# PX4/disparity_to_point_cloud

Measured on NVIDIA B200. Metric: Mpixels/s disparity->PointCloud2, higher is better.
Workload: dtype f64

## Files before the change

### disparity_to_point_cloud_b200/csrc/capi.cu

```cuda
#include "../../include/d2pc_b200.h"

#include <algorithm>
#include <atomic>
#include <cmath>
#include <cstdio>
#include <cstdlib>
#include <cstring>
#include <mutex>
#include <new>
#include <string>
#include <utility>
#include <vector>

#include <nvtx3/nvToolsExt.h>
#include <sys/mman.h>

#include "cloud_transform.h"
#include "crop_box.h"
#include "fusion.h"
#include "median.h"
#include "radius_outlier.h"
#include "reproject.h"
#include "score.h"
#include "voxel.h"
// ... 54 lines not shown
};

}

struct d2pc_ctx {
  d2pc_config cfg;
  int device = 0;
  int sm_count = 148;
  cudaStream_t s_h2d = nullptr, s_compute = nullptr, s_d2h = nullptr;
  double q[16];
  QParams Q;
  std::vector<Slot> slots;
  uint32_t epoch = 0;
  uint64_t launches = 0;
  std::string last_cuda_error;
  StageBufs batch;
  uint32_t *d_ticket = nullptr;
  d2pc_voxel_grid voxel;
  bool voxel_set = false;
  d2pc_radius_outlier ror;
  d2pc_crop_box box;
  d2pc_cloud_transform xform;
  DevBuf d_fuse_in[4], d_container, d_combined, d_fused;
  PinBuf h_fused, h_combined;
  DevBuf d_score_in, d_score_out[2];
  PinBuf h_score[2];
  DevBuf d_color_in, d_color_out, d_color_lut;
  PinBuf h_color;
  PinBuf h_stage;
  bool color_lut_ready = false;
  cudaEvent_t ev_fuse = nullptr;
  int rows_per_unit = 0, ctas_per_sm = 0, median_strip = 0, median_variant = 0;
  bool force_scalar = false, force_generic = false;
  int compact_variant = 0, exact_variant = 0, prefetch_dist = 0, zero_numer = 0;
  int fuse_median = 0;
  int direct_out = 0;
  bool timing = false;
  std::vector<std::pair<uintptr_t, bool>> pin_cache;
  uint64_t pin_cache_gen = 0;
};

namespace {

struct NvtxRange {
  explicit NvtxRange(const char *name) { nvtxRangePushA(name); }
  ~NvtxRange() { nvtxRangePop(); }
};

std::atomic<uint64_t> g_host_gen{1};

int cuda_fail(d2pc_ctx *ctx, cudaError_t e, const char *what) {
  if (ctx) {
    ctx->last_cuda_error = std::string(what) + ": " + cudaGetErrorString(e);
  }
  if (e == cudaErrorMemoryAllocation) return D2PC_ERR_NOMEM;
  if (e == cudaErrorNoDevice || e == cudaErrorInsufficientDriver || e == cudaErrorInvalidDevice)
    return D2PC_ERR_NO_DEVICE;
  return D2PC_ERR_CUDA;
}

#define CU(ctx, call)                                      \
  do {                                                     \
    cudaError_t e__ = (call);                              \
    if (e__ != cudaSuccess) return cuda_fail(ctx, e__, #call); \
  } while (0)

int grow_dev(d2pc_ctx *ctx, DevBuf &b, size_t bytes, cudaStream_t clear_on = nullptr) {
// ... 266 lines not shown

int enqueue_reproject(d2pc_ctx *ctx, const CloudPlan &p, const FrameBatch &in, StageBufs &b, const CloudDst &dst,
                      uint32_t *ticket, cudaStream_t stream) {
  const d2pc_config &c = ctx->cfg;
  int nl = 0;
  ReprojectLaunch L;
  L.in = in.data;
  L.in_is_f32 = in.is_f32;
  L.step = in.step;
  L.frame_stride = in.frame_stride;
  L.n_frames = in.n_frames;
  L.width = in.w;
  L.height = in.h;
  L.border = c.border;
  L.scale = c.disparity_scale;
  L.out = dst.points;
  L.out_stride_bytes = dst.stride;
  L.counts = dst.counts;
  L.Q = &ctx->Q;
  L.arith_fast = c.arith_mode == D2PC_ARITH_FAST;
  L.compact = p.compact;
  L.scratch = b.scratch.p;
  L.tables = b.tables.p;
  L.ticket = ticket;
  L.sm_count = ctx->sm_count;
  L.rows_per_unit = ctx->rows_per_unit;
  L.ctas_per_sm = ctx->ctas_per_sm;
  L.force_scalar = ctx->force_scalar;
  L.force_generic = ctx->force_generic;
  L.compact_variant = ctx->compact_variant;
  L.exact_variant = ctx->exact_variant;
  L.zero_numer = ctx->zero_numer;
  L.prefetch_dist = ctx->prefetch_dist;
  if (!in.is_f32 && c.median_ksize > 1) {
    MedianLaunch M;
    M.src = in.data;
    M.dst = b.med.p;
    M.src_step = M.dst_step = in.step;
    M.src_frame_stride = M.dst_frame_stride = in.frame_stride;
    M.n_frames = in.n_frames;
    M.width = (int)in.w;
    M.height = (int)in.h;
    M.ox0 = c.border;
    M.oy0 = c.border;
    M.ow = (int)in.w - 2 * c.border;
    M.oh = (int)in.h - 2 * c.border;
    M.ksize = c.median_ksize;
    M.sm_count = ctx->sm_count;
    M.strip_rows = ctx->median_strip;
    M.variant = ctx->median_variant;
    bool zero_numer = false;
    const bool fuse = ctx->fuse_median >= 0 && M.ow > 0 && M.oh > 0 && (c.median_ksize > 3 || M.variant != 0) &&
                      reproject_fuses_with_median(L, &zero_numer);
    if (fuse) {
      M.zero_numer = zero_numer;
      M.points = dst.points;
      M.points_stride_bytes = dst.stride;
      M.Q = &ctx->Q;
      M.scale = c.disparity_scale;
    }
    CU(ctx, launch_median_u8(M, stream, &nl));
    ctx->launches += nl;
    if (fuse) return D2PC_OK;
    L.in = b.med.p;
  }
  L.epoch = L.compact ? next_epoch(ctx) : 0;
// ... 232 lines not shown
  auto fail = [&](int code) {
    d2pc_destroy(ctx);
    return code;
  };
  if (cudaSetDevice(device) != cudaSuccess) return fail(D2PC_ERR_NO_DEVICE);
  cudaDeviceGetAttribute(&ctx->sm_count, cudaDevAttrMultiProcessorCount, device);
  if (cudaStreamCreateWithFlags(&ctx->s_h2d, cudaStreamNonBlocking) != cudaSuccess ||
      cudaStreamCreateWithFlags(&ctx->s_compute, cudaStreamNonBlocking) != cudaSuccess ||
      cudaStreamCreateWithFlags(&ctx->s_d2h, cudaStreamNonBlocking) != cudaSuccess ||
      cudaEventCreateWithFlags(&ctx->ev_fuse, cudaEventDisableTiming) != cudaSuccess)
    return fail(D2PC_ERR_CUDA);
  if (cudaMalloc(&ctx->d_ticket, 64) != cudaSuccess) return fail(D2PC_ERR_NOMEM);
  ctx->slots.resize(c.n_slots);
  for (auto &s : ctx->slots) {
    if (cudaEventCreateWithFlags(&s.ev_h2d, cudaEventDisableTiming) != cudaSuccess ||
        cudaEventCreateWithFlags(&s.ev_kernel, cudaEventDisableTiming) != cudaSuccess ||
        cudaEventCreateWithFlags(&s.ev_d2h, cudaEventDisableTiming) != cudaSuccess ||
        cudaStreamCreateWithFlags(&s.s_kern, cudaStreamNonBlocking) != cudaSuccess)
      return fail(D2PC_ERR_CUDA);
    if (cudaMalloc(&s.d_count, 64) != cudaSuccess) return fail(D2PC_ERR_NOMEM);
    if (cudaHostAlloc(&s.h_count, 64, cudaHostAllocDefault) != cudaSuccess) return fail(D2PC_ERR_NOMEM);
    cudaMemsetAsync(s.d_count, 0, 64, ctx->s_compute);
  }
  rc = d2pc_q_from_intrinsics(c.fx, c.fy, c.cx, c.cy, c.baseline, c.rect_width, c.rect_height, ctx->q);
  if (rc) return fail(rc);
  make_qparams(ctx->q, &ctx->Q);
  d2pc_voxel_grid_default(&ctx->voxel);
  d2pc_radius_outlier_default(&ctx->ror);
  d2pc_crop_box_default(&ctx->box);
  d2pc_cloud_transform_default(&ctx->xform);

  if (const char *v = getenv("D2PC_ROWS_PER_UNIT")) ctx->rows_per_unit = atoi(v);
  if (const char *v = getenv("D2PC_CTAS_PER_SM")) ctx->ctas_per_sm = atoi(v);
  if (const char *v = getenv("D2PC_MEDIAN_STRIP")) ctx->median_strip = atoi(v);
  if (const char *v = getenv("D2PC_EXACT_VARIANT")) ctx->exact_variant = atoi(v);

  if (c.max_width > 0 && c.max_height > 0) {
    for (auto &s : ctx->slots) {
      const size_t pitch = round_up((size_t)c.max_width * 4, kAlign);
      const uint64_t np = crop_points(c.max_width, c.max_height, c.border);
      if ((rc = grow_dev(ctx, s.d_in, pitch * c.max_height)) ||
          (rc = grow_dev(ctx, s.stages.med, pitch * c.max_height)) ||
          (rc = grow_dev(ctx, s.d_out, np * 16 + 16)) || (rc = grow_pin(ctx, s.h_out, np * 16 + 16)) ||
          (rc = grow_pin(ctx, s.h_in, (size_t)c.max_width * 4 * c.max_height)))
        return fail(rc);
    }
  }
  *out = ctx;
  return D2PC_OK;
}

void d2pc_destroy(d2pc_ctx *ctx) {
  if (!ctx) return;
  cudaSetDevice(ctx->device);
  cudaDeviceSynchronize();
  for (auto &s : ctx->slots) {
    free_pin(s.h_in), free_pin(s.h_out);
    free_dev(s.d_in), free_dev(s.d_out), free_stages(s.stages);
    for (auto &b : s.d_fuse_in) free_dev(b);
    free_dev(s.d_pre[0]), free_dev(s.d_pre[1]), free_dev(s.d_container), free_dev(s.d_combined), free_dev(s.d_fused);
    if (s.d_count) cudaFree(s.d_count);
    if (s.h_count) cudaFreeHost(s.h_count);
    if (s.ev_h2d) cudaEventDestroy(s.ev_h2d);
    if (s.ev_kernel) cudaEventDestroy(s.ev_kernel);
    if (s.ev_d2h) cudaEventDestroy(s.ev_d2h);
    if (s.ev_start) cudaEventDestroy(s.ev_start);
// ... 99 lines not shown
}
int d2pc_set_cloud_transform(d2pc_ctx *ctx, const d2pc_cloud_transform *t) {
  if (!ctx || !t || t->struct_size != sizeof(*t)) return D2PC_ERR_INVALID_ARG;
  for (float m : t->matrix)
    if (!std::isfinite(m)) return D2PC_ERR_INVALID_ARG;
  ctx->xform = *t;
  return D2PC_OK;
}
int d2pc_get_cloud_transform(const d2pc_ctx *ctx, d2pc_cloud_transform *t) {
  if (!ctx || !t) return D2PC_ERR_INVALID_ARG;
  *t = ctx->xform;
  return D2PC_OK;
}
int d2pc_set_arith_mode(d2pc_ctx *ctx, int m) {
  if (!ctx || m < 0 || m > 1) return D2PC_ERR_INVALID_ARG;
  ctx->cfg.arith_mode = m;
  return D2PC_OK;
}
int d2pc_set_tuning(d2pc_ctx *ctx, const char *key, int value) {
  if (!ctx || !key) return D2PC_ERR_INVALID_ARG;
  const std::string k(key);
  if (k == "rows_per_unit") ctx->rows_per_unit = value;
  else if (k == "ctas_per_sm") ctx->ctas_per_sm = value;
  else if (k == "median_strip") ctx->median_strip = value;
  else if (k == "median_variant") ctx->median_variant = value;
  else if (k == "force_scalar") ctx->force_scalar = value != 0;
  else if (k == "force_generic") ctx->force_generic = value != 0;
  else if (k == "force_park" || k == "compact_variant") ctx->compact_variant = value;
  else if (k == "exact_variant") ctx->exact_variant = value;
  else if (k == "zero_numer") ctx->zero_numer = value;
  else if (k == "fuse_median") ctx->fuse_median = value;
  else if (k == "direct_out") ctx->direct_out = value;
  else if (k == "prefetch_dist") ctx->prefetch_dist = value;
  else if (k == "median_ksize") {
    if (value < 1 || value > 15 || !(value & 1)) return D2PC_ERR_INVALID_ARG;
    ctx->cfg.median_ksize = value;
  } else if (k == "border") {
    if (value < 0) return D2PC_ERR_INVALID_ARG;
    ctx->cfg.border = value;
  } else if (k == "offset_x") ctx->cfg.offset_x = value;
  else if (k == "offset_y") ctx->cfg.offset_y = value;
  else if (k == "fuse_rule") {
    if (value < 0 || value > 7) return D2PC_ERR_INVALID_ARG;
    ctx->cfg.fuse_rule = value;
  } else if (k == "fuse_median_ksize") {
    if (value < 1 || value > 15 || !(value & 1)) return D2PC_ERR_INVALID_ARG;
    ctx->cfg.fuse_median_ksize = value;
  } else if (k == "fuse_crop_left") ctx->cfg.fuse_crop_left = value;
  else if (k == "fuse_crop_right") ctx->cfg.fuse_crop_right = value;
  else if (k == "fuse_crop_top") ctx->cfg.fuse_crop_top = value;
  else if (k == "fuse_crop_bottom") ctx->cfg.fuse_crop_bottom = value;
  else return D2PC_ERR_INVALID_ARG;
  return D2PC_OK;
}

int d2pc_submit_mono8(d2pc_ctx *ctx, int slot, const uint8_t *data, uint32_t w, uint32_t h, uint32_t step) {
  return submit_common(ctx, slot, data, w, h, step, false);
}
int d2pc_submit_f32(d2pc_ctx *ctx, int slot, const float *disp, uint32_t w, uint32_t h, uint32_t step) {
  return submit_common(ctx, slot, disp, w, h, step, true);
}

int d2pc_wait(d2pc_ctx *ctx, int slot, d2pc_cloud *out) {
  if (!ctx || slot < 0 || slot >= (int)ctx->slots.size()) return D2PC_ERR_INVALID_ARG;
  Slot &s = ctx->slots[slot];
  if (!s.pending) return D2PC_ERR_NOT_READY;
// ... 740 lines not shown
```

### disparity_to_point_cloud_b200/csrc/reproject.cu

```cuda
#include "reproject.h"

#include <algorithm>
#include <cmath>

#include "reproject_math.cuh"

namespace d2pc {

namespace {

constexpr int kWarpsPerCta = 4;
constexpr int kThreads = kWarpsPerCta * 32;
constexpr int kSegCols = 128;

struct FastDiv {
  uint32_t magic, shift;
};
static FastDiv make_fastdiv(uint32_t d) {
  FastDiv f{0u, 0u};
  if (d <= 1) return f;
  uint32_t s = 0;
  while ((1ull << (s + 1)) < d) ++s;
  f.shift = 32 + s;
  f.magic = (uint32_t)(((1ull << f.shift) + d - 1) / d);
  return f;
}
__device__ __forceinline__ uint32_t fastdiv(uint32_t n, FastDiv f) {
  return f.shift == 0u ? n : (uint32_t)(((unsigned long long)n * f.magic) >> f.shift);
}

struct ReprojArgs {
  const uint8_t *in;
  size_t step, frame_stride;
  float4 *out;
  size_t out_frame_stride;
  uint32_t *counts;
  int n_frames, width, height, border, cw, ch;
  int rows_per_unit, n_seg, n_rb;
  uint32_t units_per_frame, total_units;
  FastDiv div_upf, div_nseg;
  float scale;
  unsigned long long *tile_desc;
  uint32_t *ticket;
  uint32_t epoch, tiles_per_frame;
  const double *xtab, *ytab;
  uint32_t d_sure_bits;
  int band_rows, cw_pad, band_groups, group_rows;
  int prefetch_dist;
  QParams Q;
};

enum { kMathRect0 = 0, kMathRectW = 1, kMathGeneric = 2, kMathFast = 3, kMathRect0M = 4, kMathRect0Z = 5 };
#define D2PC_IS_RECT(m) ((m) == kMathRect0 || (m) == kMathRectW || (m) == kMathRect0M || (m) == kMathRect0Z)
#define D2PC_IS_GUARD(m) ((m) == kMathRect0 || (m) == kMathRect0Z)

__device__ __forceinline__ float4 ld_stream_f4(const float4 *p) {
  float4 v;
  asm volatile("ld.global.cs.v4.f32 {%0,%1,%2,%3}, [%4];" : "=f"(v.x), "=f"(v.y), "=f"(v.z), "=f"(v.w) : "l"(p));
  return v;
}
__device__ __forceinline__ void st_stream_f4(float4 *p, const float4 &v) {
  asm volatile("st.global.cs.v4.f32 [%0], {%1,%2,%3,%4};" ::"l"(p), "f"(v.x), "f"(v.y), "f"(v.z), "f"(v.w) : "memory");
}

__device__ __forceinline__ void st_stream_f4_if(float4 *p, const float4 &v, bool pred) {
  asm volatile(
      "{\n\t.reg .pred q;\n\tsetp.ne.b32 q, %5, 0;\n\t@q st.global.cs.v4.f32 [%0], {%1,%2,%3,%4};\n\t}" ::"l"(p),
      "f"(v.x), "f"(v.y), "f"(v.z), "f"(v.w), "r"((int)pred)
      : "memory");
}

__device__ __forceinline__ uint32_t store_ranked(float4 *out, uint32_t pos, const float4 &p, bool keep, int lane,
                                                 uint32_t lt_mask) {
  const uint32_t bal = __ballot_sync(0xffffffffu, keep);
  if (bal == 0xffffffffu) {
    __stcs(out + (pos + (uint32_t)lane), p);
    return pos + 32u;
  }
  if (bal == 0u) return pos;
  if (keep) __stcs(out + (pos + (uint32_t)__popc(bal & lt_mask)), p);
  return pos + (uint32_t)__popc(bal);
}

__device__ __forceinline__ uint32_t store_ranked_tight(float4 *out, uint32_t pos, const float4 &p, bool keep) {
  uint32_t lt;
// ... 37 lines not shown
}

template <int kMath>
__device__ __forceinline__ void points_of4(const QParams &Q, const double (&xd)[4], double yd, uint32_t xslow,
                                           uint32_t yslow, int u0, int v, const float (&d)[4], float4 (&p)[4]) {
  if constexpr (D2PC_IS_RECT(kMath)) {
    bool slow[4];
    const bool ys = (yslow & 1u) != 0u, yz = (yslow & 2u) != 0u;
#pragma unroll
    for (int k = 0; k < 4; ++k) {
      if constexpr (kMath == kMathRect0Z)
        p[k] = reproject_exact_rectified<true, true, true>(Q, xd[k], yd, ys || ((xslow >> k) & 1u),
                                                           yz || ((xslow >> (4 + k)) & 1u), d[k], slow[k]);
      else
        p[k] = reproject_exact_rectified<kMath != kMathRectW, kMath == kMathRect0>(Q, xd[k], yd,
                                                                                   ys || ((xslow >> k) & 1u), false,
                                                                                   d[k], slow[k]);
    }
    if (__builtin_expect(slow[0] || slow[1] || slow[2] || slow[3], 0)) {
#pragma unroll
      for (int k = 0; k < 4; ++k)
        if (slow[k]) p[k] = reproject_exact_slow(Q.q, u0 + 32 * k, v, d[k]);
    }
  } else if constexpr (kMath == kMathGeneric) {
    bool slow[4];
    const double dv = (double)v;
#pragma unroll
    for (int k = 0; k < 4; ++k) p[k] = reproject_exact_generic_guarded(Q.q, (double)(u0 + 32 * k), dv, d[k], slow[k]);
    if (__builtin_expect(slow[0] || slow[1] || slow[2] || slow[3], 0)) {
#pragma unroll
      for (int k = 0; k < 4; ++k)
        if (slow[k]) p[k] = reproject_exact_slow(Q.q, u0 + 32 * k, v, d[k]);
    }
  } else {
#pragma unroll
    for (int k = 0; k < 4; ++k) p[k] = reproject_fast(Q.qf, u0 + 32 * k, v, d[k]);
  }
}

__device__ __forceinline__ uint32_t midpoint_distance(double q) {
  return ((uint32_t)__double2loint(q) & 0x1fffffffu) - 0x0ffffff0u;
}
__device__ __forceinline__ void points_of4_keep(const QParams &Q, const double (&xd)[4], double yd, bool numer_slow,
                                                int u0, int v, const float (&d)[4], uint32_t sure_lo,
                                                uint32_t fast_span, float4 (&p)[4], bool (&keep)[4]) {
  bool rare = numer_slow;
  uint32_t cls[4];
#pragma unroll
  for (int k = 0; k < 4; ++k) {
    const uint32_t mag = __float_as_uint(d[k]) & 0x7fffffffu;
    cls[k] = mag - sure_lo;
    rare |= (cls[k] >= fast_span) && ((mag - 1u) < 0x7f7fffffu);
    const double w = __fma_rn(Q.q32, (double)d[k], 0.0);
    const double r = rcp_1ulp_inrange(w);
    const double qx = __dmul_rn(xd[k], r), qy = __dmul_rn(yd, r), qz = __dmul_rn(Q.zd, r);
    rare |= min(midpoint_distance(qx), min(midpoint_distance(qy), midpoint_distance(qz))) <= 0x20u;
    p[k].x = __double2float_rn(qx);
    p[k].y = __double2float_rn(qy);
    p[k].z = __double2float_rn(qz);
    p[k].w = 1.0f;
  }
  if (__builtin_expect(rare, 0)) {
#pragma unroll
    for (int k = 0; k < 4; ++k) {
      p[k] = reproject_exact_slow(Q.q, u0 + 32 * k, v, d[k]);
      keep[k] = (cls[k] < fast_span) || point_is_finite(p[k]);
    }
  } else {
#pragma unroll
    for (int k = 0; k < 4; ++k) keep[k] = cls[k] < fast_span;
  }
}

template <int kMath>
__device__ __forceinline__ float4 point_of(const QParams &Q, int u, int v, float d) {
  if constexpr (D2PC_IS_RECT(kMath)) {
    const double xd = rect_axis_const(u, Q.q03), yd = rect_axis_const(v, Q.q13);
    bool slow;
    float4 p = reproject_exact_rectified<kMath != kMathRectW, D2PC_IS_GUARD(kMath), kMath == kMathRect0Z>(
        Q, xd, yd, rect_axis_slow_t<kMath == kMathRect0Z>(xd) || rect_axis_slow_t<kMath == kMathRect0Z>(yd) || Q.zd_slow,
        rect_axis_zero(xd) || rect_axis_zero(yd), d, slow);
    if (__builtin_expect(slow, 0)) p = reproject_exact_slow(Q.q, u, v, d);
    return p;
  } else if constexpr (kMath == kMathGeneric) {
    return reproject_exact_generic(Q.q, u, v, d);
  } else {
    return reproject_fast(Q.qf, u, v, d);
  }
}

template <typename InT, bool kVec, int kMath, int kMinBlocks>
__global__ void __launch_bounds__(kThreads, kMinBlocks) reproject_crop_kernel(const __grid_constant__ ReprojArgs a) {
  __shared__ __align__(16) float stage[kWarpsPerCta][2][kSegCols];
  const int lane = threadIdx.x & 31;
  const int wic = threadIdx.x >> 5;
  const QParams &Q = a.Q;

  const uint32_t unit = blockIdx.x * kWarpsPerCta + wic;
  if (unit >= a.total_units) return;
  const uint32_t f = fastdiv(unit, a.div_upf);
  const uint32_t rem = unit - f * a.units_per_frame;
  const int rb = (int)fastdiv(rem, a.div_nseg);
  const int seg = rem - rb * a.n_seg;
  const int c_base = seg * kSegCols;
  const int r_base = rb * a.rows_per_unit;
  const int rows = min(a.rows_per_unit, a.ch - r_base);

  if constexpr (kVec && sizeof(InT) == 4) {
    if (a.prefetch_dist > 0 && lane < a.rows_per_unit) {
      const uint32_t u2 = unit + (uint32_t)a.prefetch_dist;
      if (u2 < a.total_units) {
        const uint32_t f2 = fastdiv(u2, a.div_upf);
        const uint32_t rem2 = u2 - f2 * a.units_per_frame;
        const int rb2 = (int)fastdiv(rem2, a.div_nseg), seg2 = rem2 - rb2 * a.n_seg;
        const int row2 = rb2 * a.rows_per_unit + lane;
        const int cols2 = min(kSegCols, ((a.cw - seg2 * kSegCols) + 3) & ~3);
        if (row2 < a.ch)
          asm volatile("cp.async.bulk.prefetch.L2.global [%0], %1;" ::"l"(a.in + (size_t)f2 * a.frame_stride +
                                                                        (size_t)(a.border + row2) * a.step +
                                                                        (size_t)(a.border + seg2 * kSegCols) * 4),
                       "r"((uint32_t)cols2 * 4u)
                       : "memory");
      }
    }
  }

  double xd[4];
  uint32_t xslow = 0;
  double yd_lane = 0.0;
  if constexpr (D2PC_IS_RECT(kMath)) {
#pragma unroll
    for (int k = 0; k < 4; ++k) {
      xd[k] = rect_axis_const(a.border + c_base + 32 * k + lane, Q.q03);
      xslow |= rect_axis_slow_t<kMath == kMathRect0Z>(xd[k]) ? (1u << k) : 0u;
      if constexpr (kMath == kMathRect0Z) xslow |= rect_axis_zero(xd[k]) ? (16u << k) : 0u;
    }
    if (Q.zd_slow) xslow = 0xfu;
    yd_lane = rect_axis_const(a.border + r_base + lane, Q.q13);
  } else {
#pragma unroll
    for (int k = 0; k < 4; ++k) xd[k] = 0.0;
  }
  double gcx[kMath == kMathGeneric ? 4 : 1][4];
  if constexpr (kMath == kMathGeneric) {
#pragma unroll
    for (int k = 0; k < 4; ++k) {
      const double du = (double)(a.border + c_base + 32 * k + lane);
#pragma unroll
      for (int i = 0; i < 4; ++i) {
        gcx[k][i] = __dmul_rn(Q.q[4 * i], du);
        asm volatile("" : "+d"(gcx[k][i]));
      }
    }
  }

  const uint8_t *in_row = a.in + (size_t)f * a.frame_stride + (size_t)(a.border + r_base) * a.step;
  float4 *out_row = a.out + (size_t)f * a.out_frame_stride + (size_t)r_base * a.cw;

  for (int r = 0; r < rows; r += 2, in_row += 2 * a.step, out_row += 2 * (size_t)a.cw) {
    float dd[2][4];
    if constexpr (kVec) {
      const int c4 = c_base + 4 * lane;
#pragma unroll
      for (int j = 0; j < 2; ++j) {
        if (r + j < rows && c4 < a.cw) {
          const float4 v = load4<InT>(in_row + (size_t)j * a.step, a.border + c4, a.scale);
          *reinterpret_cast<float4 *>(&stage[wic][j][4 * lane]) = v;
        }
      }
      __syncwarp();
#pragma unroll
      for (int j = 0; j < 2; ++j)
#pragma unroll
        for (int k = 0; k < 4; ++k) dd[j][k] = stage[wic][j][32 * k + lane];
      __syncwarp();
    } else {
#pragma unroll
      for (int j = 0; j < 2; ++j) {
#pragma unroll
        for (int k = 0; k < 4; ++k) {
          const int c = c_base + 32 * k + lane;
          dd[j][k] = (r + j < rows && c < a.cw) ? load1<InT>(in_row + (size_t)j * a.step, a.border + c, a.scale) : 1.0f;
        }
      }
    }
#pragma unroll
    for (int j = 0; j < 2; ++j) {
      if (r + j >= rows) break;
      double yd = 0.0;
      uint32_t yslow = 0;
      if constexpr (D2PC_IS_RECT(kMath)) {
        yd = __shfl_sync(0xffffffffu, yd_lane, r + j);
        yslow = rect_axis_slow_t<kMath == kMathRect0Z>(yd) ? 1u : 0u;
        if constexpr (kMath == kMathRect0Z) yslow |= rect_axis_zero(yd) ? 2u : 0u;
      }
      float4 p[4];
      if constexpr (kMath == kMathGeneric) {
        const int v = a.border + r_base + r + j, u0 = a.border + c_base + lane;
        const double dv = (double)v;
        double gry[4];
#pragma unroll
        for (int i = 0; i < 4; ++i) gry[i] = __dmul_rn(Q.q[4 * i + 1], dv);
        bool slow[4];
#pragma unroll
        for (int k = 0; k < 4; ++k) p[k] = reproject_exact_generic_hoisted(Q.q, gcx[k], gry, dd[j][k], slow[k]);
        if (__builtin_expect(slow[0] || slow[1] || slow[2] || slow[3], 0)) {
#pragma unroll
          for (int k = 0; k < 4; ++k)
            if (slow[k]) p[k] = reproject_exact_slow(Q.q, u0 + 32 * k, v, dd[j][k]);
        }
      } else {
        points_of4<kMath>(Q, xd, yd, xslow, yslow, a.border + c_base + lane, a.border + r_base + r + j, dd[j], p);
      }
      float4 *o = out_row + (size_t)j * a.cw + c_base + lane;
#pragma unroll
      for (int k = 0; k < 4; ++k)
        if (c_base + 32 * k + lane < a.cw) st_stream_f4(o + 32 * k, p[k]);
    }
  }
}

constexpr int kCWarps = 8;
constexpr int kCThreads = kCWarps * 32;
constexpr int kCIter = 4;
constexpr int kTileUnits = kCWarps * kCIter;
constexpr int kTilePts = kTileUnits * kSegCols;
constexpr size_t kCompactSmem = (size_t)kTilePts * 12 + (size_t)kCWarps * kSegCols * 4;
constexpr uint32_t kFlagAggregate = 1, kFlagPrefix = 2;

__device__ __forceinline__ unsigned long long desc_pack(uint32_t epoch, uint32_t flag, uint32_t value) {
  return ((unsigned long long)epoch << 34) | ((unsigned long long)flag << 32) | value;
}
__device__ __forceinline__ unsigned long long ld_relaxed_u64(const unsigned long long *p) {
  unsigned long long v;
  asm volatile("ld.relaxed.gpu.global.u64 %0, [%1];" : "=l"(v) : "l"(p) : "memory");
  return v;
}
__device__ __forceinline__ void st_relaxed_u64(unsigned long long *p, unsigned long long v) {
  asm volatile("st.relaxed.gpu.global.u64 [%0], %1;" ::"l"(p), "l"(v) : "memory");
}

__global__ void rect_tables_kernel(double q03, double q13, int width, int height, bool zero_ok, double *xtab,
                                   double *ytab) {
  const int i = blockIdx.x * blockDim.x + threadIdx.x;
  const double qnan = __longlong_as_double(0x7ff8000000000000ll);
  if (i < width + kSegCols) {
// ... 421 lines not shown
    const int r_lo = g * a.group_rows, r_hi = min(r_lo + a.group_rows, R);
    const int u0 = a.border + sgm * kSegCols + lane;
    double xd[4];
    uint32_t xslow = Q.zd_slow ? 0xfu : 0u;
#pragma unroll
    for (int k = 0; k < 4; ++k) {
      xd[k] = rect_axis_const(u0 + 32 * k, Q.q03);
      xslow |= rect_axis_slow_t<kZN>(xd[k]) ? (1u << k) : 0u;
    }
    for (int r = r_lo; r < r_hi; ++r) {
      const double yd = syd[r];
      const bool yslow = ((uint32_t)__double2hiint(yd) & 0x7ff00000u) == 0x7ff00000u;
      const float *dp = &sd[r * cwp + sgm * kSegCols + lane];
      float dd[4];
#pragma unroll
      for (int k = 0; k < 4; ++k) dd[k] = dp[32 * k];
      float4 p[4];
      bool kp[4];
      points_of4_keep(Q, xd, yd, yslow || xslow != 0u, u0, a.border + row0 + r, dd, sure_lo, fast_span, p, kp);
      uint32_t pos = unit_off[r * n_seg + sgm];
      if (__all_sync(0xffffffffu, kp[0] && kp[1] && kp[2] && kp[3])) {
        float4 *o = out_f + pos + lane;
#pragma unroll
        for (int k = 0; k < 4; ++k) __stcs(o + 32 * k, p[k]);
      } else {
#pragma unroll
        for (int k = 0; k < 4; ++k) pos = store_ranked_tight(out_f, pos, p[k], kp[k]);
      }
    }
  }
}


template <typename K>
cudaError_t launch_compact(K kernel, const ReprojArgs &a, int grid, cudaStream_t s) {
  cudaError_t e = cudaFuncSetAttribute(kernel, cudaFuncAttributeMaxDynamicSharedMemorySize, (int)kCompactSmem);
  if (e != cudaSuccess) return e;
  kernel<<<grid, kCThreads, kCompactSmem, s>>>(a);
  return cudaGetLastError();
}

template <typename InT, int kMath>
cudaError_t launch_typed(const ReprojArgs &a, bool vec, bool compact, int grid, int min_blocks, cudaStream_t s) {
  if (compact) {
    if constexpr (D2PC_IS_GUARD(kMath)) {
      if (a.d_sure_bits != 0 && a.band_rows > 0) {
        constexpr bool kZN = kMath == kMathRect0Z;
        const size_t smem = (size_t)a.band_rows * a.cw_pad * sizeof(float);
        auto kern = !vec ? reproject_compact_band_kernel<InT, false, 3, 8, kZN>
                         : (min_blocks == 3 ? reproject_compact_band_kernel<InT, true, 3, 8, kZN>
                                            : reproject_compact_band_kernel<InT, true, 4, 8, kZN>);
        if (smem > 48 * 1024) {
          cudaError_t e = cudaFuncSetAttribute(kern, cudaFuncAttributeMaxDynamicSharedMemorySize, (int)smem);
          if (e != cudaSuccess) return e;
        }
        kern<<<grid, kCThreads, smem, s>>>(a);
        return cudaGetLastError();
      }
    }
    return vec ? launch_compact(reproject_compact_kernel<InT, true, kMath>, a, grid, s)
               : launch_compact(reproject_compact_kernel<InT, false, kMath>, a, grid, s);
  } else if (vec) {
    switch (min_blocks) {
      case 4: reproject_crop_kernel<InT, true, kMath, 4><<<grid, kThreads, 0, s>>>(a); break;
      case 6: reproject_crop_kernel<InT, true, kMath, 6><<<grid, kThreads, 0, s>>>(a); break;
      case 8: reproject_crop_kernel<InT, true, kMath, 8><<<grid, kThreads, 0, s>>>(a); break;
      default: reproject_crop_kernel<InT, true, kMath, 7><<<grid, kThreads, 0, s>>>(a); break;
    }
  } else {
    reproject_crop_kernel<InT, false, kMath, 6><<<grid, kThreads, 0, s>>>(a);
  }
  return cudaGetLastError();
}

}

void make_qparams(const double q[16], QParams *out) {
  QParams P{};
  for (int i = 0; i < 16; ++i) {
    P.q[i] = q[i];
    P.qf[i] = (float)q[i];
  }
  auto bits = [](double x) {
    uint64_t b;
    memcpy(&b, &x, 8);
    return b;
  };
  auto pzero = [&](double x) { return bits(x) == 0; };
  auto fin = [](double x) { return x == x && x - x == 0.0; };
  const double a32 = q[14] < 0 ? -q[14] : q[14];
  const bool rect = q[0] == 1.0 && pzero(q[1]) && pzero(q[2]) && pzero(q[4]) && q[5] == 1.0 && pzero(q[6]) &&
                    pzero(q[8]) && pzero(q[9]) && pzero(q[10]) && pzero(q[12]) && pzero(q[13]) && fin(q[3]) &&
                    fin(q[7]) && fin(q[11]) && fin(q[15]) && fin(q[14]) && a32 > 1e-30 && a32 < 1e30;
  P.rectified = rect ? 1 : 0;
// ... 22 lines not shown

static uint64_t compact_tiles_per_frame(long cw, long ch) {
  const uint64_t n_seg = (uint64_t)((cw + kSegCols - 1) / kSegCols);
  return (n_seg * (uint64_t)ch + kTileUnits - 1) / kTileUnits;
}

size_t reproject_scratch_bytes(uint32_t n_frames, uint32_t width, uint32_t height, int border) {
  const long cw = (long)width - 2L * border, ch = (long)height - 2L * border;
  const uint64_t tiles = (cw > 0 && ch > 0) ? std::max<uint64_t>(compact_tiles_per_frame(cw, ch), (uint64_t)ch) : 0;
  return (size_t)(tiles * n_frames * 8 + 256);
}
size_t reproject_table_bytes(uint32_t width, uint32_t height) { return ((size_t)width + kSegCols + height) * 8 + 64; }

static int select_math(const ReprojectLaunch &L) {
  const QParams &Q = *L.Q;
  auto zero_column = [&]() {
    const double c = std::nearbyint(-Q.q03);
    return c >= 0.0 && c < (double)L.width && (float)(c + Q.q03) == 0.0f;
  };
  const bool zero_numer = L.zero_numer > 0 || (L.zero_numer == 0 && zero_column());
  return L.arith_fast ? kMathFast
         : (Q.rectified && !L.force_generic
                ? (Q.q33_zero ? (L.exact_variant == 1 ? kMathRect0M : (zero_numer ? kMathRect0Z : kMathRect0)) : kMathRectW)
                : kMathGeneric);
}

bool reproject_fuses_with_median(const ReprojectLaunch &L, bool *zero_numer) {
  if (!L.Q || L.compact || L.Q->zd_slow) return false;
  const int math = select_math(L);
  if (zero_numer) *zero_numer = math == kMathRect0Z;
  return D2PC_IS_GUARD(math);
}

cudaError_t launch_reproject(const ReprojectLaunch &L, cudaStream_t stream, int *launches) {
  const long cw = (long)L.width - 2L * L.border, ch = (long)L.height - 2L * L.border;
  if (launches) *launches = 0;
  if (cw <= 0 || ch <= 0 || L.n_frames == 0) {
    if (L.counts && L.n_frames) {
      if (launches) *launches = 0;
      return cudaMemsetAsync(L.counts, 0, sizeof(uint32_t) * L.n_frames, stream);
    }
    return cudaSuccess;
  }
  ReprojArgs a{};
  a.in = static_cast<const uint8_t *>(L.in);
  a.step = L.step;
  a.frame_stride = L.frame_stride;
  a.out = reinterpret_cast<float4 *>(L.out);
  a.out_frame_stride = L.out_stride_bytes / 16;
  a.counts = L.counts;
  a.n_frames = (int)L.n_frames;
  a.width = (int)L.width;
  a.height = (int)L.height;
  a.border = L.border;
  a.cw = (int)cw;
  a.ch = (int)ch;
  a.scale = L.scale;
  a.Q = *L.Q;

  const int esz = L.in_is_f32 ? 4 : 1;
  const size_t valign = L.in_is_f32 ? 16 : 4;
  const bool vec = (reinterpret_cast<uintptr_t>(L.in) % valign == 0) && (L.step % valign == 0) &&
                   (L.frame_stride % valign == 0) && ((size_t)L.border * esz % valign == 0) &&
                   (cw % 4 == 0 || L.border >= 3) && !L.force_scalar;

  const int math = select_math(L);
  const bool compact = L.compact;

  int grid;
  a.n_seg = (int)((cw + kSegCols - 1) / kSegCols);
  if (compact) {
    a.units_per_frame = (uint32_t)a.n_seg * (uint32_t)ch;
    a.tiles_per_frame = (uint32_t)compact_tiles_per_frame(cw, ch);
    a.tile_desc = static_cast<unsigned long long *>(L.scratch);
    double *tabs = static_cast<double *>(L.tables);
    a.xtab = tabs;
    a.ytab = tabs + L.width + kSegCols;
    a.ticket = L.ticket;
    a.epoch = L.epoch;
    const uint64_t total = (uint64_t)a.tiles_per_frame * L.n_frames;
    if (total > 0xffffffffull) return cudaErrorInvalidValue;
    grid = (int)total;
    cudaError_t e = cudaMemsetAsync(a.ticket, 0, sizeof(uint32_t), stream);
    if (e != cudaSuccess) return e;
    if (D2PC_IS_GUARD(math) && !a.Q.zd_slow && L.compact_variant != 1) {
      const double aq32 = a.Q.q32 < 0 ? -a.Q.q32 : a.Q.q32;
      auto mag = [](double x) { return x < 0 ? -x : x; };
      double max_numer = mag(a.Q.zd);
      max_numer = std::max(max_numer, mag(a.Q.q03) + (double)L.width + 1.0);
      max_numer = std::max(max_numer, mag(a.Q.q13) + (double)L.height + 1.0);
      double d_sure = 2.0 * max_numer * 0x1p-127 / aq32;
      if (d_sure < 0x1p-126) d_sure = 0x1p-126;
      if (d_sure < 3.0e38) {
        float fs = (float)d_sure;
        if ((double)fs < d_sure) fs = std::nextafter(fs, INFINITY);
        memcpy(&a.d_sure_bits, &fs, 4);
      }
    }
    if (a.d_sure_bits != 0 && L.compact_variant != 1) {
      a.cw_pad = a.n_seg * kSegCols;
      const size_t row_bytes = (size_t)a.cw_pad * sizeof(float);
      const int bw = kCWarps;
      int r_max = (int)std::min<size_t>((46 * 1024) / row_bytes, (size_t)kBandMaxRows);
      r_max = std::min(r_max, kBandMaxUnits / a.n_seg);
      if (r_max < 1 && row_bytes <= 200 * 1024 && a.n_seg <= kBandMaxUnits) r_max = 1;
      if (r_max > (int)ch) r_max = (int)ch;
      if (L.rows_per_unit > 0 && L.rows_per_unit < r_max) r_max = L.rows_per_unit;
      double best = -1.0;
      for (int r = r_max; r >= 1 && r >= r_max - 3; --r)
        for (int g = 1; g <= r; ++g) {
          const int gr = (r + g - 1) / g, ga = (r + gr - 1) / gr;
          const int items = a.n_seg * ga;
          const double eff = (double)items / (bw * ((items + bw - 1) / bw));
          const double score = eff * (gr / (gr + 0.6)) * (r / (r + 0.5));
          if (score > best + 1e-9) best = score, a.band_rows = r, a.band_groups = ga, a.group_rows = gr;
        }
      if (a.band_rows > 0) {
        a.tiles_per_frame = (uint32_t)((ch + a.band_rows - 1) / a.band_rows);
        const uint64_t total_b = (uint64_t)a.tiles_per_frame * L.n_frames;
        if (total_b > 0xffffffffull) return cudaErrorInvalidValue;
        grid = (int)total_b;
        a.prefetch_dist = L.prefetch_dist < 0 ? 0 : (L.prefetch_dist > 0 ? L.prefetch_dist : L.sm_count);
      }
    }
    if (a.Q.rectified && !L.arith_fast && !L.force_generic && a.band_rows == 0) {
      const int n = (int)(L.width + kSegCols > L.height ? L.width + kSegCols : L.height);
      rect_tables_kernel<<<(n + 255) / 256, 256, 0, stream>>>(a.Q.q03, a.Q.q13, (int)L.width, (int)L.height,
                                                            math == kMathRect0Z, tabs, tabs + L.width + kSegCols);
      if ((e = cudaGetLastError()) != cudaSuccess) return e;
      if (launches) *launches += 1;
    }
  } else {
    int rb = L.rows_per_unit > 0 ? L.rows_per_unit : 8;
    const uint64_t want_units = (uint64_t)L.sm_count * 32;
    while (rb > 2 && (uint64_t)a.n_seg * ((ch + rb - 1) / rb) * L.n_frames < want_units) rb >>= 1;
    if (rb > 32) rb = 32;
    rb &= ~1;
    if (rb < 2) rb = 2;
    a.rows_per_unit = rb;
    a.n_rb = (int)((ch + rb - 1) / rb);
    a.units_per_frame = (uint32_t)a.n_seg * (uint32_t)a.n_rb;
    const uint64_t total = (uint64_t)a.units_per_frame * L.n_frames;
    if (total >= 0x7fffffffull) return cudaErrorInvalidValue;
    a.total_units = (uint32_t)total;
    a.div_upf = make_fastdiv(a.units_per_frame);
    a.div_nseg = make_fastdiv((uint32_t)a.n_seg);
    grid = (int)((total + kWarpsPerCta - 1) / kWarpsPerCta);
    a.prefetch_dist = L.prefetch_dist < 0 ? 0 : (L.prefetch_dist > 0 ? std::min(L.prefetch_dist, 1 << 24) : 512);
  }
  const int min_blocks = L.ctas_per_sm > 0 ? L.ctas_per_sm : (math == kMathGeneric && !compact ? 4 : 6);
  if (launches) *launches += 1;

#define D2PC_DISPATCH(T)                                                          \
  switch (math) {                                                                 \
    case kMathRect0: return launch_typed<T, kMathRect0>(a, vec, compact, grid, min_blocks, stream); \
    case kMathRect0Z: return launch_typed<T, kMathRect0Z>(a, vec, compact, grid, min_blocks, stream); \
    case kMathRect0M: return launch_typed<T, kMathRect0M>(a, vec, compact, grid, min_blocks, stream); \
    case kMathRectW: return launch_typed<T, kMathRectW>(a, vec, compact, grid, min_blocks, stream); \
    case kMathGeneric: return launch_typed<T, kMathGeneric>(a, vec, compact, grid, min_blocks, stream); \
    default: return launch_typed<T, kMathFast>(a, vec, compact, grid, min_blocks, stream);    \
  }
  if (L.in_is_f32) {
    D2PC_DISPATCH(float)
  } else {
    D2PC_DISPATCH(uint8_t)
  }
#undef D2PC_DISPATCH
}

}
```

### disparity_to_point_cloud_b200/csrc/reproject.h

```cpp
#pragma once
#include <cstddef>
#include <cstdint>
#include <cstring>
#include <cuda_runtime.h>

namespace d2pc {

struct QParams {
  double q[16];
  double q03, q13, q32, q33;
  double zd;
  float qf[16];
  float zinf;
  uint32_t dhi_bits;
  int rectified;
  int q33_zero;
  int zd_slow;
};

struct ReprojectLaunch {
  const void *in = nullptr;
  bool in_is_f32 = true;
  size_t step = 0, frame_stride = 0;
  uint32_t n_frames = 0, width = 0, height = 0;
  int border = 40;
  float scale = 0.125f;
  uint8_t *out = nullptr;
  size_t out_stride_bytes = 0;
  uint32_t *counts = nullptr;
  const QParams *Q = nullptr;
  bool arith_fast = false;
  bool compact = false;
  void *scratch = nullptr;
  void *tables = nullptr;
  uint32_t *ticket = nullptr;
  uint32_t epoch = 1;
  int sm_count = 148;
  int rows_per_unit = 0;
  int ctas_per_sm = 0;
  bool force_scalar = false;
  bool force_generic = false;
  int exact_variant = 0;
  int zero_numer = 0;
  int compact_variant = 0;
  int prefetch_dist = 0;
};

void make_qparams(const double q[16], QParams *out);
size_t reproject_scratch_bytes(uint32_t n_frames, uint32_t width, uint32_t height, int border);
size_t reproject_table_bytes(uint32_t width, uint32_t height);
cudaError_t launch_reproject(const ReprojectLaunch &L, cudaStream_t stream, int *launches);
bool reproject_fuses_with_median(const ReprojectLaunch &L, bool *zero_numer);

}
```

Baseline: 339,100.

## Load crop tiles with TMA bulk tensor copies in the reproject kernel

Adds a TMA-based crop kernel that fetches each warp's rows-by-128-column disparity tile with cp.async.bulk.tensor into shared memory, synchronised by an mbarrier. It also issues L2 tensor prefetches for a later unit. It becomes the default for vectorised f32 input, with four rows per unit instead of eight. The aim is to replace per-lane global loads with bulk async copies. The cost is a host-side tensor-map encode on every launch and smaller work units. A probe math mode and tuning knobs are added as well.

```diff
diff --git a/disparity_to_point_cloud_b200/csrc/capi.cu b/disparity_to_point_cloud_b200/csrc/capi.cu
--- a/disparity_to_point_cloud_b200/csrc/capi.cu
+++ b/disparity_to_point_cloud_b200/csrc/capi.cu
@@ -110,7 +110,7 @@
   cudaEvent_t ev_fuse = nullptr;
   int rows_per_unit = 0, ctas_per_sm = 0, median_strip = 0, median_variant = 0;
   bool force_scalar = false, force_generic = false;
-  int compact_variant = 0, exact_variant = 0, prefetch_dist = 0, zero_numer = 0;
+  int compact_variant = 0, exact_variant = 0, prefetch_dist = 0, zero_numer = 0, crop_load = 0, crop_probe = 0;
   int fuse_median = 0;
   int direct_out = 0;
   bool timing = false;
@@ -443,6 +443,8 @@
   L.exact_variant = ctx->exact_variant;
   L.zero_numer = ctx->zero_numer;
   L.prefetch_dist = ctx->prefetch_dist;
+  L.crop_load = ctx->crop_load;
+  L.crop_probe = ctx->crop_probe != 0;
   if (!in.is_f32 && c.median_ksize > 1) {
     MedianLaunch M;
     M.src = in.data;
@@ -741,6 +743,7 @@
 
   if (const char *v = getenv("D2PC_ROWS_PER_UNIT")) ctx->rows_per_unit = atoi(v);
   if (const char *v = getenv("D2PC_CTAS_PER_SM")) ctx->ctas_per_sm = atoi(v);
+  if (const char *v = getenv("D2PC_CROP_LOAD")) ctx->crop_load = atoi(v);
   if (const char *v = getenv("D2PC_MEDIAN_STRIP")) ctx->median_strip = atoi(v);
   if (const char *v = getenv("D2PC_EXACT_VARIANT")) ctx->exact_variant = atoi(v);
 
@@ -906,6 +909,8 @@
   else if (k == "fuse_median") ctx->fuse_median = value;
   else if (k == "direct_out") ctx->direct_out = value;
   else if (k == "prefetch_dist") ctx->prefetch_dist = value;
+  else if (k == "crop_load") ctx->crop_load = value;
+  else if (k == "crop_probe") ctx->crop_probe = value;
   else if (k == "median_ksize") {
     if (value < 1 || value > 15 || !(value & 1)) return D2PC_ERR_INVALID_ARG;
     ctx->cfg.median_ksize = value;
diff --git a/disparity_to_point_cloud_b200/csrc/reproject.cu b/disparity_to_point_cloud_b200/csrc/reproject.cu
--- a/disparity_to_point_cloud_b200/csrc/reproject.cu
+++ b/disparity_to_point_cloud_b200/csrc/reproject.cu
@@ -1,4 +1,7 @@
 #include "reproject.h"
+
+#include <cuda.h>
+#include <cudaTypedefs.h>
 
 #include <algorithm>
 #include <cmath>
@@ -30,6 +33,8 @@
 }
 
 struct ReprojArgs {
+  CUtensorMap tmap;
+  bool tma;
   const uint8_t *in;
   size_t step, frame_stride;
   float4 *out;
@@ -50,7 +55,7 @@
   QParams Q;
 };
 
-enum { kMathRect0 = 0, kMathRectW = 1, kMathGeneric = 2, kMathFast = 3, kMathRect0M = 4, kMathRect0Z = 5 };
+enum { kMathRect0 = 0, kMathRectW = 1, kMathGeneric = 2, kMathFast = 3, kMathRect0M = 4, kMathRect0Z = 5, kMathProbe = 6 };
 #define D2PC_IS_RECT(m) ((m) == kMathRect0 || (m) == kMathRectW || (m) == kMathRect0M || (m) == kMathRect0Z)
 #define D2PC_IS_GUARD(m) ((m) == kMathRect0 || (m) == kMathRect0Z)
 
@@ -154,6 +159,9 @@
       for (int k = 0; k < 4; ++k)
         if (slow[k]) p[k] = reproject_exact_slow(Q.q, u0 + 32 * k, v, d[k]);
     }
+  } else if constexpr (kMath == kMathProbe) {
+#pragma unroll
+    for (int k = 0; k < 4; ++k) p[k] = make_float4(d[k], d[k], d[k], 1.0f);
   } else {
 #pragma unroll
     for (int k = 0; k < 4; ++k) p[k] = reproject_fast(Q.qf, u0 + 32 * k, v, d[k]);
@@ -211,19 +219,94 @@
   }
 }
 
+template <int kMath>
+struct CropCols {
+  double xd[4];
+  uint32_t xslow;
+  double yd_lane;
+  double gcx[kMath == kMathGeneric ? 4 : 1][4];
+};
+
+template <int kMath>
+__device__ __forceinline__ void crop_cols_init(CropCols<kMath> &c, const ReprojArgs &a, int c_base, int r_base,
+                                               int lane) {
+  const QParams &Q = a.Q;
+  c.xslow = 0;
+  c.yd_lane = 0.0;
+  if constexpr (D2PC_IS_RECT(kMath)) {
+#pragma unroll
+    for (int k = 0; k < 4; ++k) {
+      c.xd[k] = rect_axis_const(a.border + c_base + 32 * k + lane, Q.q03);
+      c.xslow |= rect_axis_slow_t<kMath == kMathRect0Z>(c.xd[k]) ? (1u << k) : 0u;
+      if constexpr (kMath == kMathRect0Z) c.xslow |= rect_axis_zero(c.xd[k]) ? (16u << k) : 0u;
+    }
+    if (Q.zd_slow) c.xslow = 0xfu;
+    c.yd_lane = rect_axis_const(a.border + r_base + lane, Q.q13);
+  } else {
+#pragma unroll
+    for (int k = 0; k < 4; ++k) c.xd[k] = 0.0;
+  }
+  if constexpr (kMath == kMathGeneric) {
+#pragma unroll
+    for (int k = 0; k < 4; ++k) {
+      const double du = (double)(a.border + c_base + 32 * k + lane);
+#pragma unroll
+      for (int i = 0; i < 4; ++i) {
+        c.gcx[k][i] = __dmul_rn(Q.q[4 * i], du);
+        asm volatile("" : "+d"(c.gcx[k][i]));
+      }
+    }
+  }
+}
+
+template <int kMath>
+__device__ __forceinline__ void crop_row_points(const ReprojArgs &a, const CropCols<kMath> &c, int c_base, int r_base,
+                                                int r, int lane, const float (&d)[4], float4 (&p)[4]) {
+  const QParams &Q = a.Q;
+  double yd = 0.0;
+  uint32_t yslow = 0;
+  if constexpr (D2PC_IS_RECT(kMath)) {
+    yd = __shfl_sync(0xffffffffu, c.yd_lane, r);
+    yslow = rect_axis_slow_t<kMath == kMathRect0Z>(yd) ? 1u : 0u;
+    if constexpr (kMath == kMathRect0Z) yslow |= rect_axis_zero(yd) ? 2u : 0u;
+  }
+  if constexpr (kMath == kMathGeneric) {
+    const int v = a.border + r_base + r, u0 = a.border + c_base + lane;
+    const double dv = (double)v;
+    double gry[4];
+#pragma unroll
+    for (int i = 0; i < 4; ++i) gry[i] = __dmul_rn(Q.q[4 * i + 1], dv);
+    bool slow[4];
+#pragma unroll
+    for (int k = 0; k < 4; ++k) p[k] = reproject_exact_generic_hoisted(Q.q, c.gcx[k], gry, d[k], slow[k]);
+    if (__builtin_expect(slow[0] || slow[1] || slow[2] || slow[3], 0)) {
+#pragma unroll
+      for (int k = 0; k < 4; ++k)
+        if (slow[k]) p[k] = reproject_exact_slow(Q.q, u0 + 32 * k, v, d[k]);
+    }
+  } else {
+    points_of4<kMath>(Q, c.xd, yd, c.xslow, yslow, a.border + c_base + lane, a.border + r_base + r, d, p);
+  }
+}
+
+__device__ __forceinline__ void crop_unit(const ReprojArgs &a, uint32_t unit, uint32_t &f, int &rb, int &seg) {
+  f = fastdiv(unit, a.div_upf);
+  const uint32_t rem = unit - f * a.units_per_frame;
+  rb = (int)fastdiv(rem, a.div_nseg);
+  seg = (int)rem - rb * a.n_seg;
+}
+
 template <typename InT, bool kVec, int kMath, int kMinBlocks>
 __global__ void __launch_bounds__(kThreads, kMinBlocks) reproject_crop_kernel(const __grid_constant__ ReprojArgs a) {
   __shared__ __align__(16) float stage[kWarpsPerCta][2][kSegCols];
   const int lane = threadIdx.x & 31;
   const int wic = threadIdx.x >> 5;
-  const QParams &Q = a.Q;
 
   const uint32_t unit = blockIdx.x * kWarpsPerCta + wic;
   if (unit >= a.total_units) return;
-  const uint32_t f = fastdiv(unit, a.div_upf);
-  const uint32_t rem = unit - f * a.units_per_frame;
-  const int rb = (int)fastdiv(rem, a.div_nseg);
-  const int seg = rem - rb * a.n_seg;
+  uint32_t f;
+  int rb, seg;
+  crop_unit(a, unit, f, rb, seg);
   const int c_base = seg * kSegCols;
   const int r_base = rb * a.rows_per_unit;
   const int rows = min(a.rows_per_unit, a.ch - r_base);
@@ -232,9 +315,9 @@
     if (a.prefetch_dist > 0 && lane < a.rows_per_unit) {
       const uint32_t u2 = unit + (uint32_t)a.prefetch_dist;
       if (u2 < a.total_units) {
-        const uint32_t f2 = fastdiv(u2, a.div_upf);
-        const uint32_t rem2 = u2 - f2 * a.units_per_frame;
-        const int rb2 = (int)fastdiv(rem2, a.div_nseg), seg2 = rem2 - rb2 * a.n_seg;
+        uint32_t f2;
+        int rb2, seg2;
+        crop_unit(a, u2, f2, rb2, seg2);
         const int row2 = rb2 * a.rows_per_unit + lane;
         const int cols2 = min(kSegCols, ((a.cw - seg2 * kSegCols) + 3) & ~3);
         if (row2 < a.ch)
@@ -247,34 +330,8 @@
     }
   }
 
-  double xd[4];
-  uint32_t xslow = 0;
-  double yd_lane = 0.0;
-  if constexpr (D2PC_IS_RECT(kMath)) {
-#pragma unroll
-    for (int k = 0; k < 4; ++k) {
-      xd[k] = rect_axis_const(a.border + c_base + 32 * k + lane, Q.q03);
-      xslow |= rect_axis_slow_t<kMath == kMathRect0Z>(xd[k]) ? (1u << k) : 0u;
-      if constexpr (kMath == kMathRect0Z) xslow |= rect_axis_zero(xd[k]) ? (16u << k) : 0u;
-    }
-    if (Q.zd_slow) xslow = 0xfu;
-    yd_lane = rect_axis_const(a.border + r_base + lane, Q.q13);
-  } else {
-#pragma unroll
-    for (int k = 0; k < 4; ++k) xd[k] = 0.0;
-  }
-  double gcx[kMath == kMathGeneric ? 4 : 1][4];
-  if constexpr (kMath == kMathGeneric) {
-#pragma unroll
-    for (int k = 0; k < 4; ++k) {
-      const double du = (double)(a.border + c_base + 32 * k + lane);
-#pragma unroll
-      for (int i = 0; i < 4; ++i) {
-        gcx[k][i] = __dmul_rn(Q.q[4 * i], du);
-        asm volatile("" : "+d"(gcx[k][i]));
-      }
-    }
-  }
+  CropCols<kMath> cols;
+  crop_cols_init(cols, a, c_base, r_base, lane);
 
   const uint8_t *in_row = a.in + (size_t)f * a.frame_stride + (size_t)(a.border + r_base) * a.step;
   float4 *out_row = a.out + (size_t)f * a.out_frame_stride + (size_t)r_base * a.cw;
@@ -309,31 +366,8 @@
 #pragma unroll
     for (int j = 0; j < 2; ++j) {
       if (r + j >= rows) break;
-      double yd = 0.0;
-      uint32_t yslow = 0;
-      if constexpr (D2PC_IS_RECT(kMath)) {
-        yd = __shfl_sync(0xffffffffu, yd_lane, r + j);
-        yslow = rect_axis_slow_t<kMath == kMathRect0Z>(yd) ? 1u : 0u;
-        if constexpr (kMath == kMathRect0Z) yslow |= rect_axis_zero(yd) ? 2u : 0u;
-      }
       float4 p[4];
-      if constexpr (kMath == kMathGeneric) {
-        const int v = a.border + r_base + r + j, u0 = a.border + c_base + lane;
-        const double dv = (double)v;
-        double gry[4];
-#pragma unroll
-        for (int i = 0; i < 4; ++i) gry[i] = __dmul_rn(Q.q[4 * i + 1], dv);
-        bool slow[4];
-#pragma unroll
-        for (int k = 0; k < 4; ++k) p[k] = reproject_exact_generic_hoisted(Q.q, gcx[k], gry, dd[j][k], slow[k]);
-        if (__builtin_expect(slow[0] || slow[1] || slow[2] || slow[3], 0)) {
-#pragma unroll
-          for (int k = 0; k < 4; ++k)
-            if (slow[k]) p[k] = reproject_exact_slow(Q.q, u0 + 32 * k, v, dd[j][k]);
-        }
-      } else {
-        points_of4<kMath>(Q, xd, yd, xslow, yslow, a.border + c_base + lane, a.border + r_base + r + j, dd[j], p);
-      }
+      crop_row_points<kMath>(a, cols, c_base, r_base, r + j, lane, dd[j], p);
       float4 *o = out_row + (size_t)j * a.cw + c_base + lane;
 #pragma unroll
       for (int k = 0; k < 4; ++k)
@@ -821,6 +855,82 @@
 }
 
 
+template <int kMath, int kMinBlocks, int kR>
+__global__ void __launch_bounds__(kThreads, kMinBlocks) reproject_crop_tma_kernel(const __grid_constant__ ReprojArgs a) {
+  __shared__ __align__(128) float box[kWarpsPerCta][kR * kSegCols];
+  __shared__ __align__(8) unsigned long long bar[kWarpsPerCta];
+  const int lane = threadIdx.x & 31;
+  const int wic = threadIdx.x >> 5;
+  const uint32_t unit = blockIdx.x * kWarpsPerCta + wic;
+  if (unit >= a.total_units) return;
+  uint32_t f;
+  int rb, seg;
+  crop_unit(a, unit, f, rb, seg);
+  const int c_base = seg * kSegCols;
+  const int r_base = rb * kR;
+  const uint64_t tmap = reinterpret_cast<uint64_t>(&a.tmap);
+  if (lane == 0) {
+    mbar_init(&bar[wic], 1);
+    asm volatile("fence.mbarrier_init.release.cluster;" ::: "memory");
+    mbar_arrive_expect_tx(&bar[wic], kR * kSegCols * 4);
+    asm volatile(
+        "cp.async.bulk.tensor.3d.shared::cluster.global.tile.mbarrier::complete_tx::bytes [%0], [%1, {%2, %3, %4}], "
+        "[%5];" ::"r"(smem_u32(box[wic])),
+        "l"(tmap), "r"(c_base), "r"(r_base), "r"((int)f), "r"(smem_u32(&bar[wic]))
+        : "memory");
+    const uint32_t u2 = unit + (uint32_t)a.prefetch_dist;
+    if (a.prefetch_dist > 0 && u2 < a.total_units) {
+      uint32_t f2;
+      int rb2, seg2;
+      crop_unit(a, u2, f2, rb2, seg2);
+      asm volatile("cp.async.bulk.prefetch.tensor.3d.L2.global.tile [%0, {%1, %2, %3}];" ::"l"(tmap),
+                   "r"(seg2 * kSegCols), "r"(rb2 * kR), "r"((int)f2)
+                   : "memory");
+    }
+  }
+  CropCols<kMath> cols;
+  crop_cols_init(cols, a, c_base, r_base, lane);
+  __syncwarp();
+  mbar_wait(&bar[wic], 0);
+
+  const float *bx = box[wic] + lane;
+  float4 *o = a.out + (size_t)f * a.out_frame_stride + (uint32_t)(r_base * a.cw + c_base + lane);
+  if (r_base + kR <= a.ch && c_base + kSegCols <= a.cw) {
+#pragma unroll
+    for (int r = 0; r < kR; ++r, o += a.cw) {
+      float d[4];
+#pragma unroll
+      for (int k = 0; k < 4; ++k) d[k] = bx[r * kSegCols + 32 * k];
+      float4 p[4];
+      crop_row_points<kMath>(a, cols, c_base, r_base, r, lane, d, p);
+#pragma unroll
+      for (int k = 0; k < 4; ++k) st_stream_f4(o + 32 * k, p[k]);
+    }
+  } else {
+    const int rows = min(kR, a.ch - r_base);
+#pragma unroll 1
+    for (int r = 0; r < rows; ++r, o += a.cw) {
+      float d[4];
+#pragma unroll
+      for (int k = 0; k < 4; ++k) d[k] = bx[r * kSegCols + 32 * k];
+      float4 p[4];
+      crop_row_points<kMath>(a, cols, c_base, r_base, r, lane, d, p);
+#pragma unroll
+      for (int k = 0; k < 4; ++k)
+        if (c_base + 32 * k + lane < a.cw) st_stream_f4(o + 32 * k, p[k]);
+    }
+  }
+}
+
+template <int kMath, int kMinBlocks>
+void launch_crop_tma(const ReprojArgs &a, int grid, cudaStream_t s) {
+  switch (a.rows_per_unit) {
+    case 4: reproject_crop_tma_kernel<kMath, kMinBlocks, 4><<<grid, kThreads, 0, s>>>(a); break;
+    case 6: reproject_crop_tma_kernel<kMath, kMinBlocks, 6><<<grid, kThreads, 0, s>>>(a); break;
+    default: reproject_crop_tma_kernel<kMath, kMinBlocks, 8><<<grid, kThreads, 0, s>>>(a); break;
+  }
+}
+
 template <typename K>
 cudaError_t launch_compact(K kernel, const ReprojArgs &a, int grid, cudaStream_t s) {
   cudaError_t e = cudaFuncSetAttribute(kernel, cudaFuncAttributeMaxDynamicSharedMemorySize, (int)kCompactSmem);
@@ -831,7 +941,19 @@
 
 template <typename InT, int kMath>
 cudaError_t launch_typed(const ReprojArgs &a, bool vec, bool compact, int grid, int min_blocks, cudaStream_t s) {
+  if constexpr (sizeof(InT) == 4) {
+    if (a.tma) {
+      switch (min_blocks) {
+        case 4: launch_crop_tma<kMath, 4>(a, grid, s); break;
+        case 6: launch_crop_tma<kMath, 6>(a, grid, s); break;
+        case 8: launch_crop_tma<kMath, 8>(a, grid, s); break;
+        default: launch_crop_tma<kMath, 7>(a, grid, s); break;
+      }
+      return cudaGetLastError();
+    }
+  }
   if (compact) {
+    if constexpr (kMath == kMathProbe) return cudaErrorInvalidValue;
     if constexpr (D2PC_IS_GUARD(kMath)) {
       if (a.d_sure_bits != 0 && a.band_rows > 0) {
         constexpr bool kZN = kMath == kMathRect0Z;
@@ -847,8 +969,9 @@
         return cudaGetLastError();
       }
     }
-    return vec ? launch_compact(reproject_compact_kernel<InT, true, kMath>, a, grid, s)
-               : launch_compact(reproject_compact_kernel<InT, false, kMath>, a, grid, s);
+    if constexpr (kMath != kMathProbe)
+      return vec ? launch_compact(reproject_compact_kernel<InT, true, kMath>, a, grid, s)
+                 : launch_compact(reproject_compact_kernel<InT, false, kMath>, a, grid, s);
   } else if (vec) {
     switch (min_blocks) {
       case 4: reproject_crop_kernel<InT, true, kMath, 4><<<grid, kThreads, 0, s>>>(a); break;
@@ -937,6 +1060,26 @@
   return D2PC_IS_GUARD(math);
 }
 
+static bool encode_crop_map(CUtensorMap *m, const ReprojectLaunch &L, long cw, long ch, int rows) {
+  static const PFN_cuTensorMapEncodeTiled_v12000 encode = [] {
+    void *fn = nullptr;
+    cudaDriverEntryPointQueryResult q;
+    return cudaGetDriverEntryPointByVersion("cuTensorMapEncodeTiled", &fn, 12000, cudaEnableDefault, &q) ==
+                       cudaSuccess &&
+                   q == cudaDriverEntryPointSuccess
+               ? reinterpret_cast<PFN_cuTensorMapEncodeTiled_v12000>(fn)
+               : nullptr;
+  }();
+  if (!encode) return false;
+  const cuuint64_t dims[3] = {(cuuint64_t)cw, (cuuint64_t)ch, (cuuint64_t)L.n_frames};
+  const cuuint64_t strides[2] = {(cuuint64_t)L.step, L.n_frames > 1 ? (cuuint64_t)L.frame_stride : (cuuint64_t)L.step * ch};
+  const cuuint32_t box[3] = {(cuuint32_t)kSegCols, (cuuint32_t)rows, 1u}, elem[3] = {1u, 1u, 1u};
+  const uint8_t *base = static_cast<const uint8_t *>(L.in) + (size_t)L.border * L.step + (size_t)L.border * 4;
+  return encode(m, CU_TENSOR_MAP_DATA_TYPE_FLOAT32, 3, const_cast<uint8_t *>(base), dims, strides, box, elem,
+                CU_TENSOR_MAP_INTERLEAVE_NONE, CU_TENSOR_MAP_SWIZZLE_NONE, CU_TENSOR_MAP_L2_PROMOTION_L2_256B,
+                CU_TENSOR_MAP_FLOAT_OOB_FILL_NONE) == CUDA_SUCCESS;
+}
+
 cudaError_t launch_reproject(const ReprojectLaunch &L, cudaStream_t stream, int *launches) {
   const long cw = (long)L.width - 2L * L.border, ch = (long)L.height - 2L * L.border;
   if (launches) *launches = 0;
@@ -969,7 +1112,7 @@
                    (L.frame_stride % valign == 0) && ((size_t)L.border * esz % valign == 0) &&
                    (cw % 4 == 0 || L.border >= 3) && !L.force_scalar;
 
-  const int math = select_math(L);
+  int math = select_math(L);
   const bool compact = L.compact;
 
   int grid;
@@ -1036,7 +1179,8 @@
       if (launches) *launches += 1;
     }
   } else {
-    int rb = L.rows_per_unit > 0 ? L.rows_per_unit : 8;
+    const bool tma_rows = vec && L.in_is_f32 && L.crop_load == 0;
+    int rb = L.rows_per_unit > 0 ? L.rows_per_unit : (tma_rows ? 4 : 8);
     const uint64_t want_units = (uint64_t)L.sm_count * 32;
     while (rb > 2 && (uint64_t)a.n_seg * ((ch + rb - 1) / rb) * L.n_frames < want_units) rb >>= 1;
     if (rb > 32) rb = 32;
@@ -1052,6 +1196,12 @@
     a.div_nseg = make_fastdiv((uint32_t)a.n_seg);
     grid = (int)((total + kWarpsPerCta - 1) / kWarpsPerCta);
     a.prefetch_dist = L.prefetch_dist < 0 ? 0 : (L.prefetch_dist > 0 ? std::min(L.prefetch_dist, 1 << 24) : 512);
+    a.tma = tma_rows && (rb == 4 || rb == 6 || rb == 8) &&
+            (uint64_t)cw * (uint64_t)ch < (1ull << 31) && encode_crop_map(&a.tmap, L, cw, ch, rb);
+  }
+  if (L.crop_probe && !compact) {
+    if (!L.in_is_f32) return cudaErrorInvalidValue;
+    math = kMathProbe;
   }
   const int min_blocks = L.ctas_per_sm > 0 ? L.ctas_per_sm : (math == kMathGeneric && !compact ? 4 : 6);
   if (launches) *launches += 1;
@@ -1066,6 +1216,7 @@
     default: return launch_typed<T, kMathFast>(a, vec, compact, grid, min_blocks, stream);    \
   }
   if (L.in_is_f32) {
+    if (math == kMathProbe) return launch_typed<float, kMathProbe>(a, vec, compact, grid, min_blocks, stream);
     D2PC_DISPATCH(float)
   } else {
     D2PC_DISPATCH(uint8_t)
diff --git a/disparity_to_point_cloud_b200/csrc/reproject.h b/disparity_to_point_cloud_b200/csrc/reproject.h
--- a/disparity_to_point_cloud_b200/csrc/reproject.h
+++ b/disparity_to_point_cloud_b200/csrc/reproject.h
@@ -44,6 +44,8 @@
   int zero_numer = 0;
   int compact_variant = 0;
   int prefetch_dist = 0;
+  int crop_load = 0;
+  bool crop_probe = false;
 };
 
 void make_qparams(const double q[16], QParams *out);
```

Result: faster. 358,700 (median of 6 runs) (+5.8%).
